# PinataFarms/FEARTracker

Hardware: NVIDIA H100
Metric: FEAR-XS frames/sec (track + decode, batch 256 per GPU) (higher is better)
Workload: dtype f32

## Files before the change

### feartracker_b200/csrc/kernels_tc.cuh

```cuda
#pragma once
#include <cuda_runtime.h>
#include <stdlib.h>

#include <initializer_list>

#include "tc_common.cuh"

namespace fear {
namespace tc {

constexpr int kCorrChunk = 32;
constexpr int kCorrABytes = 128 * 128;
constexpr int kCorrBBytes = 64 * 128;
constexpr int kTcThreads = 288;
constexpr int kTcConsumers = 256;

__device__ __forceinline__ void consumer_sync() { asm volatile("bar.sync 1, 256;" ::: "memory"); }

constexpr int kCorrStages = 3;
constexpr int kCorrStageBytes = kCorrABytes + 2 * kCorrBBytes;
constexpr int kCorrSmemBytes = kCorrStages * kCorrStageBytes + 1024  + 256 ;

__global__ void __launch_bounds__(kTcThreads, 1)
corr_tc_kernel(const __grid_constant__ CUtensorMap tmA, const __grid_constant__ CUtensorMap tmB,
               float* __restrict__ cat, int z_mod) {
  extern __shared__ uint8_t smem_raw[];
  uint8_t* smem = smem_raw + ((1024u - (smem_u32(smem_raw) & 1023u)) & 1023u);
  uint64_t* full = reinterpret_cast<uint64_t*>(smem + kCorrStages * kCorrStageBytes);
  uint64_t* empty = full + kCorrStages;
  const int warp = threadIdx.x >> 5, lane = threadIdx.x & 31;
  constexpr int kChunks = 256 / kCorrChunk;
  if (threadIdx.x == 0) {
    prefetch_tmap(&tmA);
    prefetch_tmap(&tmB);
    for (int s = 0; s < kCorrStages; ++s) {
      mbar_init(&full[s], 1);
      mbar_init(&empty[s], 8);
    }
    fence_mbar_init();
  }
  __syncthreads();
  pdl_trigger();
  pdl_wait();
  const int frame = blockIdx.x >> 1, half = blockIdx.x & 1;
  const int arow = frame * 256 + half * 128;
  auto st_x = [&](int s) { return smem + s * kCorrStageBytes; };
  auto st_z = [&](int s) { return smem + s * kCorrStageBytes + kCorrABytes; };

  if (warp == 8) {
    if (lane == 0) {
      const int brow = z_mod ? (frame % z_mod) * 64 : 0;
      for (int c = 0; c < kChunks; ++c) {
        const int stage = c % kCorrStages;
        mbar_wait_backoff(&empty[stage], (uint32_t)(((c / kCorrStages) & 1) ^ 1));
        mbar_arrive_expect_tx(&full[stage], kCorrABytes + kCorrBBytes);
        tma_load_2d(st_x(stage), &tmA, &full[stage], c * kCorrChunk, arow);
        tma_load_2d(st_z(stage), &tmB, &full[stage], c * kCorrChunk, brow);
      }
    }
    return;
  }
  const int wg = warp >> 2, r0 = wg * 64 + (warp & 3) * 16 + (lane >> 2), t = lane & 3;
  float accm[32], accc[32];
#pragma unroll
  for (int i = 0; i < 32; ++i) accm[i] = accc[i] = 0.f;
  for (int c = 0; c < kChunks; ++c) {
    const int stage = c % kCorrStages;
    mbar_wait(&full[stage], (uint32_t)((c / kCorrStages) & 1));
    float4* zh = reinterpret_cast<float4*>(st_z(stage));
    float4* zl = reinterpret_cast<float4*>(st_z(stage) + kCorrBBytes);
#pragma unroll
    for (int i = 0; i < kCorrBBytes / 16 / kTcConsumers; ++i) {
      const float4 v = zh[threadIdx.x + i * kTcConsumers];
      float4 h, l;
      split_tf32_trunc(v.x, h.x, l.x);
      split_tf32_trunc(v.y, h.y, l.y);
      split_tf32_trunc(v.z, h.z, l.z);
      split_tf32_trunc(v.w, h.w, l.w);
      zh[threadIdx.x + i * kTcConsumers] = h;
      zl[threadIdx.x + i * kTcConsumers] = l;
    }
    fence_proxy_async_smem();
    consumer_sync();
    uint32_t hi[4][4], lo[4][4];
    load_a_frags(st_x(stage), r0, t, hi, lo);
    const uint32_t bh = smem_u32(zh), bl = smem_u32(zl);
    wg_fence();
#pragma unroll
    for (int j = 0; j < 4; ++j) mma3<64>(accm, accc, hi[j], lo[j], bh + j * 32, bl + j * 32);
    wg_commit();
    wg_wait();
    __syncwarp();
    if (lane == 0) mbar_arrive(&empty[stage]);
  }
  float* out = cat + (long long)(arow + r0) * 320 + 256 + 2 * t;
#pragma unroll
  for (int i = 0; i < 8; ++i) {
    *reinterpret_cast<float2*>(out + 8 * i) = make_float2(accm[4 * i] + accc[4 * i], accm[4 * i + 1] + accc[4 * i + 1]);
    *reinterpret_cast<float2*>(out + 8 * 320 + 8 * i) =
        make_float2(accm[4 * i + 2] + accc[4 * i + 2], accm[4 * i + 3] + accc[4 * i + 3]);
  }
}

inline int init_pw();

inline int init() {
  int dev = 0;
  if (cudaGetDevice(&dev) != cudaSuccess) return -1;
  cudaDeviceProp p;
  if (cudaGetDeviceProperties(&p, dev) != cudaSuccess) return -1;
  DeviceState& st = dev_state();
  st.num_sms = p.multiProcessorCount;
  st.inited = true;
  if (resolve_driver()) return 0;
  if (cudaFuncSetAttribute(corr_tc_kernel, cudaFuncAttributeMaxDynamicSharedMemorySize, kCorrSmemBytes) != cudaSuccess) {
    cudaGetLastError();
    return 0;
  }
  if (init_pw()) return 0;
  st.tc_ready = true;
  return 0;
}

inline int launch_corr(cudaStream_t s, const float* zt, int Bz, float* cat, int B, int groups) {
  if (!available()) return -20;
  CUtensorMap tmA, tmB;
  const int frames = B * groups;
  int r;
  r = make_tmap_2d(&tmA, cat, (uint64_t)frames * 256, 320, 320, 128, kCorrChunk);
  if (r) return r;
  r = make_tmap_2d(&tmB, zt, (uint64_t)Bz * 64, 256, 256, 64, kCorrChunk);
  if (r) return r;
  if (launch_pdl(corr_tc_kernel, dim3(frames * 2), dim3(kTcThreads), kCorrSmemBytes, s, tmA, tmB, cat, Bz == 1 ? 0 : B) !=
      cudaSuccess)
    return -23;
  return 0;
}

struct PwParams {
  const float* bias;
  const float* R;
  float* C;
  int ldr, ldc;
  int M, N, num_n_tiles, num_chunks, last_ksteps, relu, stages, stage_bytes;
  int dw_relu, dw_bias;
  int box_bytes;
};

template <int NT, int DWK, int MW = 16>
__global__ void __launch_bounds__(kTcThreads, 1)
pw_tc_kernel(const __grid_constant__ CUtensorMap tmA, const __grid_constant__ CUtensorMap tmWh,
             const __grid_constant__ CUtensorMap tmWl, const __grid_constant__ CUtensorMap tmDW,
             const __grid_constant__ CUtensorMap tmDB, const PwParams p) {
  extern __shared__ uint8_t smem_raw[];
  uint8_t* smem = smem_raw + ((1024u - (smem_u32(smem_raw) & 1023u)) & 1023u);
  const int S = p.stages;
  uint64_t* full = reinterpret_cast<uint64_t*>(smem + S * p.stage_bytes);
  uint64_t* empty = full + S;
  const int warp = threadIdx.x >> 5, lane = threadIdx.x & 31;
  constexpr int w_bytes = NT * 128;
  if (threadIdx.x == 0) {
    prefetch_tmap(&tmA);
    prefetch_tmap(&tmWh);
    prefetch_tmap(&tmWl);
    for (int s = 0; s < S; ++s) {
      mbar_init(&full[s], 1);
      mbar_init(&empty[s], 8);
    }
    fence_mbar_init();
  }
  __syncthreads();
  pdl_trigger();
  pdl_wait();

  const int mt = blockIdx.x / p.num_n_tiles, nt = blockIdx.x - mt * p.num_n_tiles;
  auto a_tile = [&](int s) { return smem + s * p.stage_bytes; };
  auto w_hi = [&](int s) { return smem + s * p.stage_bytes + kCorrABytes; };
  auto w_lo = [&](int s) { return w_hi(s) + w_bytes; };
  auto dw_box = [&](int s) { return w_lo(s) + w_bytes; };
  auto dw_wts = [&](int s) { return dw_box(s) + p.box_bytes; };
  auto dw_bia = [&](int s) { return dw_wts(s) + DWK * DWK * 128; };

  if (warp == 8) {
    if (lane == 0) {
      constexpr int th = 128 / MW, tpf = MW / th;
      for (int c = 0; c < p.num_chunks; ++c) {
        const int stage = c % S;
        mbar_wait_backoff(&empty[stage], (uint32_t)(((c / S) & 1) ^ 1));
        if constexpr (DWK > 0) {
          mbar_arrive_expect_tx(&full[stage], 2 * w_bytes + p.box_bytes + DWK * DWK * 128 + (p.dw_bias ? 128 : 0));
          tma_load_4d(dw_box(stage), &tmA, &full[stage], c * 32, -(DWK / 2), (mt % tpf) * th - DWK / 2, mt / tpf);
          tma_load_2d(dw_wts(stage), &tmDW, &full[stage], c * 32, 0);
          if (p.dw_bias) tma_load_2d(dw_bia(stage), &tmDB, &full[stage], c * 32, 0);
        } else {
          mbar_arrive_expect_tx(&full[stage], kCorrABytes + 2 * w_bytes);
          tma_load_2d(a_tile(stage), &tmA, &full[stage], c * 32, mt * 128);
        }
        tma_load_2d(w_hi(stage), &tmWh, &full[stage], c * 32, nt * NT);
        tma_load_2d(w_lo(stage), &tmWl, &full[stage], c * 32, nt * NT);
      }
    }
    return;
  }

  const int wg = warp >> 2, r0 = wg * 64 + (warp & 3) * 16 + (lane >> 2), t = lane & 3;
  float accm[NT / 2], accc[NT / 2];
#pragma unroll
  for (int i = 0; i < NT / 2; ++i) accm[i] = accc[i] = 0.f;
  for (int c = 0; c < p.num_chunks; ++c) {
    const int stage = c % S;
    mbar_wait(&full[stage], (uint32_t)((c / S) & 1));
    if constexpr (DWK > 0) {
      constexpr int K = DWK, TX = 8, NIN = TX + K - 1, IW = MW + K - 1, PXN = MW / TX;
      typedef unsigned long long U2;
      const int c2 = threadIdx.x & 15, pos = threadIdx.x >> 4;
      const int x0 = (pos % PXN) * TX, y0 = pos / PXN;
      const U2* in2 = reinterpret_cast<const U2*>(dw_box(stage)) + (y0 * IW + x0) * 16 + c2;
      const U2* w2 = reinterpret_cast<const U2*>(dw_wts(stage)) + c2;
      const U2 bias2 = p.dw_bias ? reinterpret_cast<const U2*>(dw_bia(stage))[c2] : 0ull;
      U2 acc[TX];
#pragma unroll
      for (int i = 0; i < TX; ++i) acc[i] = bias2;
#pragma unroll
      for (int ky = 0; ky < K; ++ky) {
        U2 v[NIN];
#pragma unroll
        for (int i = 0; i < NIN; ++i) v[i] = in2[(ky * IW + i) * 16];
#pragma unroll
        for (int kx = 0; kx < K; ++kx) {
          const U2 k = w2[(ky * K + kx) * 16];
#pragma unroll
          for (int i = 0; i < TX; ++i) ffma2(acc[i], v[i + kx], k);
        }
      }
      uint8_t* at = a_tile(stage);
#pragma unroll
      for (int i = 0; i < TX; ++i) {
        float2 v = make_float2(__uint_as_float((uint32_t)acc[i]), __uint_as_float((uint32_t)(acc[i] >> 32)));
        if (p.dw_relu) {
          v.x = fmaxf(v.x, 0.f);
          v.y = fmaxf(v.y, 0.f);
        }
        const int R = y0 * MW + x0 + i;
        *reinterpret_cast<float2*>(at + R * 128 + (((c2 >> 1) ^ (R & 7)) << 4) + ((c2 & 1) << 3)) = v;
      }
      consumer_sync();
    }
    uint32_t hi[4][4], lo[4][4];
    load_a_frags(a_tile(stage), r0, t, hi, lo);
    const uint32_t bh = smem_u32(w_hi(stage)), bl = smem_u32(w_lo(stage));
    const int ksteps = (c == p.num_chunks - 1) ? p.last_ksteps : 4;
    wg_fence();
#pragma unroll
    for (int j = 0; j < 4; ++j)
      if (j < ksteps) mma3<NT>(accm, accc, hi[j], lo[j], bh + j * 32, bl + j * 32);
    wg_commit();
    wg_wait();
    __syncwarp();
    if (lane == 0) mbar_arrive(&empty[stage]);
  }

  const int n0 = nt * NT + 2 * t;
#pragma unroll
  for (int hrow = 0; hrow < 2; ++hrow) {
    const long long grow = (long long)mt * 128 + r0 + hrow * 8;
    if (grow >= p.M) continue;
#pragma unroll
    for (int i = 0; i < NT / 8; ++i) {
      const int col = n0 + 8 * i;
      if (col >= p.N) continue;
      float2 o = make_float2(accm[4 * i + 2 * hrow] + accc[4 * i + 2 * hrow], accm[4 * i + 2 * hrow + 1] + accc[4 * i + 2 * hrow + 1]);
      float2 b = p.bias ? __ldg(reinterpret_cast<const float2*>(p.bias + col)) : make_float2(0.f, 0.f);
      if (p.R) {
        const float2 rr = __ldg(reinterpret_cast<const float2*>(p.R + grow * p.ldr + col));
        b.x += rr.x;
        b.y += rr.y;
      }
      o.x += b.x;
      o.y += b.y;
      if (p.relu) {
        o.x = fmaxf(o.x, 0.f);
        o.y = fmaxf(o.y, 0.f);
      }
      *reinterpret_cast<float2*>(p.C + grow * p.ldc + col) = o;
    }
  }
}

constexpr int kPwMaxSmem = 232448 - 1024;
constexpr int kPwMaxStages = 3;

inline int pw_tile_n(int N) {
  const int Np = (N + 15) & ~15;
  const int tiles = (Np + 127) / 128;
  const int need = (Np + tiles - 1) / tiles;
  for (int nt : {16, 32, 48, 64, 96, 112, 128})
    if (nt >= need) return nt;
  return 0;
}

inline bool pw_supported(int cin, int cout) { return available() && cin % 8 == 0 && cout % 8 == 0; }

#define FEAR_PW_FOR_NT(X) X(16) X(32) X(48) X(64) X(96) X(112) X(128)

constexpr int kPwNarrowNT = 32;
inline int pw_tile_n_one_chunk(int N) {
  const int Np = (N + 15) & ~15;
  const int tiles = (Np + kPwNarrowNT - 1) / kPwNarrowNT;
  const int need = (Np + tiles - 1) / tiles;
  return need <= 16 ? 16 : 32;
}

inline int init_pw() {
  cudaError_t e = cudaSuccess;
#define FEAR_PW_ATTR(NT_)                                                                                                  \
  if (e == cudaSuccess) e = cudaFuncSetAttribute(pw_tc_kernel<NT_, 0>, cudaFuncAttributeMaxDynamicSharedMemorySize, kPwMaxSmem);     \
  if (e == cudaSuccess) e = cudaFuncSetAttribute(pw_tc_kernel<NT_, 3, 16>, cudaFuncAttributeMaxDynamicSharedMemorySize, kPwMaxSmem); \
  if (e == cudaSuccess) e = cudaFuncSetAttribute(pw_tc_kernel<NT_, 5, 16>, cudaFuncAttributeMaxDynamicSharedMemorySize, kPwMaxSmem); \
  if (e == cudaSuccess) e = cudaFuncSetAttribute(pw_tc_kernel<NT_, 3, 32>, cudaFuncAttributeMaxDynamicSharedMemorySize, kPwMaxSmem); \
  if (e == cudaSuccess) e = cudaFuncSetAttribute(pw_tc_kernel<NT_, 5, 32>, cudaFuncAttributeMaxDynamicSharedMemorySize, kPwMaxSmem);
  FEAR_PW_FOR_NT(FEAR_PW_ATTR)
#undef FEAR_PW_ATTR
  if (e != cudaSuccess) {
    cudaGetLastError();
    return -1;
  }
  return 0;
}

inline int launch_pw(cudaStream_t s, const float* A, int lda, const float* w_hi, const float* w_lo, const float* bias,
                     const float* R, int ldr, float* C, int ldc, int M, int N, int K, int relu) {
  if (!available()) return -20;
  PwParams p;
  p.bias = bias;
  p.R = R;
  p.C = C;
  p.ldr = ldr;
  p.ldc = ldc;
  p.M = M;
  p.N = N;
  p.num_chunks = (K + 31) / 32;
  const int NT = p.num_chunks == 1 ? pw_tile_n_one_chunk(N) : pw_tile_n(N);
  if (!NT) return -21;
  p.num_n_tiles = (((N + 15) & ~15) + NT - 1) / NT;
  p.last_ksteps = ((K - 32 * (p.num_chunks - 1)) + 7) / 8;
  p.relu = relu;
  p.dw_relu = p.dw_bias = p.box_bytes = 0;
  p.stage_bytes = kCorrABytes + 2 * NT * 128;
  p.stages = p.num_chunks < kPwMaxStages ? p.num_chunks : kPwMaxStages;
  CUtensorMap tmA, tmWh, tmWl;
  int r = make_tmap_2d(&tmA, A, (uint64_t)M, (uint64_t)K, (uint64_t)lda, 128, 32);
  if (r) return r;
  r = make_tmap_2d(&tmWh, w_hi, (uint64_t)N, (uint64_t)K, (uint64_t)K, NT, 32);
  if (r) return r;
  r = make_tmap_2d(&tmWl, w_lo, (uint64_t)N, (uint64_t)K, (uint64_t)K, NT, 32);
  if (r) return r;
  const int tiles = ((M + 127) / 128) * p.num_n_tiles;
  const size_t smem_bytes = (size_t)p.stages * p.stage_bytes + 1024 + 256;
  cudaError_t e = cudaErrorInvalidValue;
  switch (NT) {
#define FEAR_PW_CASE(NT_)                                                                                                     \
  case NT_:                                                                                                                   \
    e = launch_pdl(pw_tc_kernel<NT_, 0>, dim3(tiles), dim3(kTcThreads), smem_bytes, s, tmA, tmWh, tmWl, tmA, tmA, p); \
    break;
    FEAR_PW_FOR_NT(FEAR_PW_CASE)
#undef FEAR_PW_CASE
  }
  return e == cudaSuccess ? 0 : -23;
}

inline int launch_pw_dw(cudaStream_t s, const float* X, int B, int dw_k, const float* dw_w, const float* dw_b, int dw_relu,
                        const float* w_hi, const float* w_lo, const float* bias, const float* R, int ldr, float* C,
                        int ldc, int N, int K, int relu, int map_w = 16) {
  if (!available()) return -20;
  if ((dw_k != 3 && dw_k != 5) || K % 4 || (map_w != 16 && map_w != 32)) return 1;
  PwParams p;
  const int M = B * map_w * map_w;
  p.bias = bias;
  p.R = R;
  p.C = C;
  p.ldr = ldr;
  p.ldc = ldc;
  p.M = M;
  p.N = N;
  p.num_chunks = (K + 31) / 32;
  const int NT = pw_tile_n(N);
  if (!NT) return 1;
  p.num_n_tiles = (((N + 15) & ~15) + NT - 1) / NT;
  p.last_ksteps = ((K - 32 * (p.num_chunks - 1)) + 7) / 8;
  p.relu = relu;
  p.dw_relu = dw_relu;
  p.dw_bias = dw_b != nullptr;
  const int ih = 128 / map_w + dw_k - 1, iw = map_w + dw_k - 1;
  p.box_bytes = ih * iw * 128;
  p.stage_bytes = (kCorrABytes + 2 * NT * 128 + p.box_bytes + dw_k * dw_k * 128 + 128 + 1023) & ~1023;
  p.stages = p.num_chunks < 2 ? 1 : 2;
  const size_t smem_bytes = (size_t)p.stages * p.stage_bytes + 1024 + 256;
  if ((int)smem_bytes > kPwMaxSmem) return 1;
  CUtensorMap tmX, tmWh, tmWl, tmDW, tmDB;
  int r = make_tmap_nhwc(&tmX, X, (uint64_t)B, (uint64_t)map_w, (uint64_t)map_w, (uint64_t)K, 32, iw, ih);
  if (r) return r;
  r = make_tmap_2d(&tmWh, w_hi, (uint64_t)N, (uint64_t)K, (uint64_t)K, NT, 32);
  if (r) return r;
  r = make_tmap_2d(&tmWl, w_lo, (uint64_t)N, (uint64_t)K, (uint64_t)K, NT, 32);
  if (r) return r;
  r = make_tmap_2d_plain(&tmDW, dw_w, (uint64_t)dw_k * dw_k, (uint64_t)K, dw_k * dw_k, 32);
  if (r) return r;
  if (dw_b) {
    r = make_tmap_2d_plain(&tmDB, dw_b, 1, (uint64_t)K, 1, 32);
    if (r) return r;
  } else {
    tmDB = tmDW;
  }
  const int tiles = (M / 128) * p.num_n_tiles;
  cudaError_t e = cudaErrorInvalidValue;
#define FEAR_PW_DW_LAUNCH(NT_, K_, MW_) \
  e = launch_pdl(pw_tc_kernel<NT_, K_, MW_>, dim3(tiles), dim3(kTcThreads), smem_bytes, s, tmX, tmWh, tmWl, tmDW, tmDB, p)
  switch (NT) {
#define FEAR_PW_CASE(NT_)                                \
  case NT_:                                              \
    if (map_w == 16) {                                   \
      if (dw_k == 5) FEAR_PW_DW_LAUNCH(NT_, 5, 16);      \
      else FEAR_PW_DW_LAUNCH(NT_, 3, 16);                \
    } else {                                             \
      if (dw_k == 5) FEAR_PW_DW_LAUNCH(NT_, 5, 32);      \
      else FEAR_PW_DW_LAUNCH(NT_, 3, 32);                \
    }                                                    \
    break;
    FEAR_PW_FOR_NT(FEAR_PW_CASE)
#undef FEAR_PW_CASE
  }
#undef FEAR_PW_DW_LAUNCH
  return e == cudaSuccess ? 0 : -23;
}

}
}
```

### feartracker_b200/csrc/tc_common.cuh

```cuda
#pragma once
#include <cuda.h>
#include <cuda_runtime.h>
#include <stdint.h>
#include <string.h>

#include <mutex>
#include <set>
#include <string>
#include <unordered_map>

namespace fear {
namespace tc {

typedef CUresult (*PFN_encodeTiled)(CUtensorMap*, CUtensorMapDataType, cuuint32_t, void*, const cuuint64_t*,
                                    const cuuint64_t*, const cuuint32_t*, const cuuint32_t*, CUtensorMapInterleave,
                                    CUtensorMapSwizzle, CUtensorMapL2promotion, CUtensorMapFloatOOBfill);

inline PFN_encodeTiled& encode_fn() {
  static PFN_encodeTiled fn = nullptr;
  return fn;
}

inline int resolve_driver() {
  if (encode_fn()) return 0;
  void* p = nullptr;
  cudaDriverEntryPointQueryResult q;
  cudaError_t e = cudaGetDriverEntryPoint("cuTensorMapEncodeTiled", &p, cudaEnableDefault, &q);
  if (e != cudaSuccess || q != cudaDriverEntryPointSuccess || !p) return -10;
  encode_fn() = (PFN_encodeTiled)p;
  return 0;
}

struct DeviceState {
  bool inited = false;
  bool tc_ready = false;
  int num_sms = 0;
  std::set<const void*> attrs;
};
inline std::mutex& state_mutex() {
  static std::mutex m;
  return m;
}
inline DeviceState& dev_state() {
  static DeviceState st[64];
  int d = 0;
  cudaGetDevice(&d);
  return st[d & 63];
}
inline bool available() { return dev_state().tc_ready; }
inline int num_sms() { return dev_state().num_sms; }
inline bool attr_needed(const void* fn) {
  std::lock_guard<std::mutex> lock(state_mutex());
  return dev_state().attrs.insert(fn).second;
}

struct TmapKey {
  uint64_t v[16];
  bool operator==(const TmapKey& o) const { return memcmp(v, o.v, sizeof(v)) == 0; }
};
struct TmapKeyHash {
  size_t operator()(const TmapKey& k) const {
    uint64_t h = 1469598103934665603ull;
    for (uint64_t x : k.v) {
      h ^= x;
      h *= 1099511628211ull;
    }
    return (size_t)h;
  }
};
inline int encode_cached(CUtensorMap* m, CUtensorMapDataType dt, uint32_t rank, const void* base, const cuuint64_t* dims,
                         const cuuint64_t* strides, const cuuint32_t* box, CUtensorMapSwizzle sw,
                         CUtensorMapL2promotion promo) {
  if (resolve_driver()) return -10;
  static thread_local std::unordered_map<TmapKey, CUtensorMap, TmapKeyHash> cache;
  TmapKey k;
  memset(&k, 0, sizeof(k));
  k.v[0] = (uint64_t)(uintptr_t)base;
  k.v[1] = ((uint64_t)dt << 32) | ((uint64_t)rank << 16) | ((uint64_t)sw << 8) | (uint64_t)promo;
  for (uint32_t i = 0; i < rank; ++i) {
    k.v[2 + i] = dims[i];
    k.v[7 + i] = (i + 1 < rank) ? strides[i] : 0;
    k.v[12 + (i >> 1)] |= (uint64_t)box[i] << (32 * (i & 1));
  }
  auto it = cache.find(k);
  if (it != cache.end()) {
    *m = it->second;
    return 0;
  }
  cuuint32_t estr[5] = {1, 1, 1, 1, 1};
  CUresult r = encode_fn()(m, dt, rank, const_cast<void*>(base), dims, strides, box, estr, CU_TENSOR_MAP_INTERLEAVE_NONE, sw,
                           promo, CU_TENSOR_MAP_FLOAT_OOB_FILL_NONE);
  if (r != CUDA_SUCCESS) return -11;
  if (cache.size() > 8192) cache.clear();
  cache.emplace(k, *m);
  return 0;
}

inline int make_tmap_2d(CUtensorMap* m, const float* base, uint64_t rows, uint64_t cols, uint64_t pitch_floats,
                        uint32_t box_rows, uint32_t box_cols) {
  cuuint64_t dims[2] = {cols, rows};
  cuuint64_t strides[1] = {pitch_floats * sizeof(float)};
  cuuint32_t box[2] = {box_cols, box_rows};
  CUtensorMapSwizzle sw = (box_cols * 4 == 128)  ? CU_TENSOR_MAP_SWIZZLE_128B
                          : (box_cols * 4 == 64) ? CU_TENSOR_MAP_SWIZZLE_64B
                                                 : CU_TENSOR_MAP_SWIZZLE_NONE;
  return encode_cached(m, CU_TENSOR_MAP_DATA_TYPE_FLOAT32, 2, base, dims, strides, box, sw,
                       CU_TENSOR_MAP_L2_PROMOTION_L2_256B);
}

inline int make_tmap_nhwc(CUtensorMap* m, const float* base, uint64_t B, uint64_t H, uint64_t W, uint64_t C,
                          uint32_t box_c, uint32_t box_w, uint32_t box_h,
                          CUtensorMapSwizzle sw = CU_TENSOR_MAP_SWIZZLE_NONE) {
  cuuint64_t dims[4] = {C, W, H, B};
  cuuint64_t strides[3] = {C * sizeof(float), W * C * sizeof(float), H * W * C * sizeof(float)};
  cuuint32_t box[4] = {box_c, box_w, box_h, 1};
  return encode_cached(m, CU_TENSOR_MAP_DATA_TYPE_FLOAT32, 4, base, dims, strides, box, sw,
                       CU_TENSOR_MAP_L2_PROMOTION_L2_128B);
}

inline int make_tmap_3d(CUtensorMap* m, CUtensorMapDataType dt, const void* base, uint64_t d0, uint64_t d1, uint64_t d2,
                        uint64_t stride1_bytes, uint64_t stride2_bytes, uint32_t b0, uint32_t b1, uint32_t b2) {
  cuuint64_t dims[3] = {d0, d1, d2};
  cuuint64_t strides[2] = {stride1_bytes, stride2_bytes};
  cuuint32_t box[3] = {b0, b1, b2};
  return encode_cached(m, dt, 3, base, dims, strides, box, CU_TENSOR_MAP_SWIZZLE_NONE, CU_TENSOR_MAP_L2_PROMOTION_L2_128B);
}

inline int make_tmap_2d_plain(CUtensorMap* m, const float* base, uint64_t rows, uint64_t cols, uint32_t box_rows,
                              uint32_t box_cols) {
  cuuint64_t dims[2] = {cols, rows};
  cuuint64_t strides[1] = {cols * sizeof(float)};
  cuuint32_t box[2] = {box_cols, box_rows};
  return encode_cached(m, CU_TENSOR_MAP_DATA_TYPE_FLOAT32, 2, base, dims, strides, box, CU_TENSOR_MAP_SWIZZLE_NONE,
                       CU_TENSOR_MAP_L2_PROMOTION_L2_128B);
}

inline bool& pdl_enabled() {
  static bool on = true;
  return on;
}
template <typename... KArgs, typename... Args>
inline cudaError_t launch_pdl(void (*kern)(KArgs...), dim3 grid, dim3 block, size_t smem, cudaStream_t s, Args&&... args) {
  cudaLaunchConfig_t cfg = {};
  cfg.gridDim = grid;
  cfg.blockDim = block;
  cfg.dynamicSmemBytes = smem;
  cfg.stream = s;
  cudaLaunchAttribute attr[1];
  attr[0].id = cudaLaunchAttributeProgrammaticStreamSerialization;
  attr[0].val.programmaticStreamSerializationAllowed = 1;
  cudaStreamCaptureStatus cap = cudaStreamCaptureStatusNone;
  const bool use = pdl_enabled() && cudaStreamIsCapturing(s, &cap) == cudaSuccess && cap == cudaStreamCaptureStatusNone;
  cfg.attrs = attr;
  cfg.numAttrs = use ? 1 : 0;
  return cudaLaunchKernelEx(&cfg, kern, static_cast<KArgs>(args)...);
}

__device__ __forceinline__ uint32_t smem_u32(const void* p) { return (uint32_t)__cvta_generic_to_shared(p); }

__device__ __forceinline__ bool elect_one() {
  uint32_t pred = 0;
  asm volatile(
      "{\n\t"
      ".reg .pred P;\n\t"
      "elect.sync _|P, 0xffffffff;\n\t"
      "selp.u32 %0, 1, 0, P;\n\t"
      "}\n"
      : "=r"(pred));
  return pred != 0;
}

__device__ __forceinline__ void mbar_init(uint64_t* bar, uint32_t count) {
  asm volatile("mbarrier.init.shared::cta.b64 [%0], %1;" ::"r"(smem_u32(bar)), "r"(count) : "memory");
}
__device__ __forceinline__ void fence_mbar_init() { asm volatile("fence.mbarrier_init.release.cluster;" ::: "memory"); }
__device__ __forceinline__ void mbar_arrive(uint64_t* bar) {
  asm volatile("mbarrier.arrive.shared::cta.b64 _, [%0];" ::"r"(smem_u32(bar)) : "memory");
}
__device__ __forceinline__ void mbar_arrive_expect_tx(uint64_t* bar, uint32_t bytes) {
  asm volatile("mbarrier.arrive.expect_tx.shared::cta.b64 _, [%0], %1;" ::"r"(smem_u32(bar)), "r"(bytes) : "memory");
}
__device__ __forceinline__ bool mbar_try_wait(uint64_t* bar, uint32_t parity) {
  uint32_t ok;
  asm volatile(
      "{\n\t"
      ".reg .pred P;\n\t"
      "mbarrier.try_wait.parity.shared::cta.b64 P, [%1], %2;\n\t"
      "selp.u32 %0, 1, 0, P;\n\t"
      "}\n"
      : "=r"(ok)
      : "r"(smem_u32(bar)), "r"(parity)
      : "memory");
  return ok != 0;
}
__device__ __forceinline__ void mbar_wait(uint64_t* bar, uint32_t parity) {
#pragma unroll 1
  for (uint32_t spin = 0; spin < (1u << 26); ++spin)
    if (mbar_try_wait(bar, parity)) return;
  __trap();
}

__device__ __forceinline__ void mbar_wait_backoff(uint64_t* bar, uint32_t parity) {
  if (mbar_try_wait(bar, parity)) return;
#pragma unroll 1
  for (uint32_t spin = 0; spin < (1u << 24); ++spin) {
    __nanosleep(64);
    if (mbar_try_wait(bar, parity)) return;
  }
  __trap();
}

__device__ __forceinline__ void fence_proxy_async_smem() { asm volatile("fence.proxy.async.shared::cta;" ::: "memory"); }

__device__ __forceinline__ void prefetch_tmap(const CUtensorMap* m) {
  asm volatile("prefetch.tensormap [%0];" ::"l"(reinterpret_cast<uint64_t>(m)) : "memory");
}
__device__ __forceinline__ void tma_load_2d(void* smem_dst, const CUtensorMap* m, uint64_t* bar, int32_t c0, int32_t c1) {
  asm volatile(
      "cp.async.bulk.tensor.2d.shared::cluster.global.mbarrier::complete_tx::bytes [%0], [%1, {%3, %4}], [%2];"
      ::"r"(smem_u32(smem_dst)), "l"(reinterpret_cast<uint64_t>(m)), "r"(smem_u32(bar)), "r"(c0), "r"(c1)
      : "memory");
}
__device__ __forceinline__ void tma_load_3d(void* smem_dst, const CUtensorMap* m, uint64_t* bar, int32_t c0, int32_t c1,
                                            int32_t c2) {
  asm volatile(
      "cp.async.bulk.tensor.3d.shared::cluster.global.mbarrier::complete_tx::bytes [%0], [%1, {%3, %4, %5}], [%2];"
      ::"r"(smem_u32(smem_dst)), "l"(reinterpret_cast<uint64_t>(m)), "r"(smem_u32(bar)), "r"(c0), "r"(c1), "r"(c2)
      : "memory");
}
__device__ __forceinline__ void tma_load_4d(void* smem_dst, const CUtensorMap* m, uint64_t* bar, int32_t c0, int32_t c1,
                                            int32_t c2, int32_t c3) {
  asm volatile(
      "cp.async.bulk.tensor.4d.shared::cluster.global.mbarrier::complete_tx::bytes [%0], [%1, {%3, %4, %5, %6}], [%2];"
      ::"r"(smem_u32(smem_dst)), "l"(reinterpret_cast<uint64_t>(m)), "r"(smem_u32(bar)), "r"(c0), "r"(c1), "r"(c2),
      "r"(c3)
      : "memory");
}
__device__ __forceinline__ void tma_prefetch_4d(const CUtensorMap* m, int32_t c0, int32_t c1, int32_t c2, int32_t c3) {
  asm volatile("cp.async.bulk.prefetch.tensor.4d.L2.global.tile [%0, {%1, %2, %3, %4}];" ::"l"(reinterpret_cast<uint64_t>(m)),
               "r"(c0), "r"(c1), "r"(c2), "r"(c3)
               : "memory");
}
__device__ __forceinline__ void tma_store_2d(const CUtensorMap* m, const void* smem_src, int32_t c0, int32_t c1) {
  asm volatile("cp.async.bulk.tensor.2d.global.shared::cta.bulk_group [%0, {%2, %3}], [%1];" ::"l"(
                   reinterpret_cast<uint64_t>(m)),
               "r"(smem_u32(smem_src)), "r"(c0), "r"(c1)
               : "memory");
}
__device__ __forceinline__ void tma_store_commit() { asm volatile("cp.async.bulk.commit_group;" ::: "memory"); }
template <int N>
__device__ __forceinline__ void tma_store_wait_read() {
  asm volatile("cp.async.bulk.wait_group.read %0;" ::"n"(N) : "memory");
}
template <int N>
__device__ __forceinline__ void tma_store_wait() {
  asm volatile("cp.async.bulk.wait_group %0;" ::"n"(N) : "memory");
}

struct __align__(16) F4 {
  unsigned long long lo, hi;
};
__device__ __forceinline__ void ffma2(unsigned long long& acc, unsigned long long a, unsigned long long b) {
  const float x = fmaf(__uint_as_float((uint32_t)a), __uint_as_float((uint32_t)b), __uint_as_float((uint32_t)acc));
  const float y = fmaf(__uint_as_float((uint32_t)(a >> 32)), __uint_as_float((uint32_t)(b >> 32)), __uint_as_float((uint32_t)(acc >> 32)));
  acc = (unsigned long long)__float_as_uint(x) | ((unsigned long long)__float_as_uint(y) << 32);
}
__device__ __forceinline__ unsigned long long pack2(uint32_t lo, uint32_t hi) {
  return (unsigned long long)lo | ((unsigned long long)hi << 32);
}
__device__ __forceinline__ float4 f4_to_float4(const F4& v) {
  float4 r;
  r.x = __uint_as_float((unsigned)(v.lo & 0xffffffffull));
  r.y = __uint_as_float((unsigned)(v.lo >> 32));
  r.z = __uint_as_float((unsigned)(v.hi & 0xffffffffull));
  r.w = __uint_as_float((unsigned)(v.hi >> 32));
  return r;
}

__device__ __forceinline__ void pdl_trigger() { asm volatile("griddepcontrol.launch_dependents;" ::: "memory"); }
__device__ __forceinline__ void pdl_wait() { asm volatile("griddepcontrol.wait;" ::: "memory"); }

__device__ __forceinline__ void wg_fence() { asm volatile("wgmma.fence.sync.aligned;" ::: "memory"); }
__device__ __forceinline__ void wg_commit() { asm volatile("wgmma.commit_group.sync.aligned;" ::: "memory"); }
__device__ __forceinline__ void wg_wait() { asm volatile("wgmma.wait_group.sync.aligned 0;" ::: "memory"); }

#define FEAR_WG_D8(d, o) "+f"(d[o]), "+f"(d[o + 1]), "+f"(d[o + 2]), "+f"(d[o + 3]), "+f"(d[o + 4]), "+f"(d[o + 5]), "+f"(d[o + 6]), "+f"(d[o + 7])
template <int N>
__device__ __forceinline__ void wgmma_tf32(float* d, const uint32_t (&a)[4], uint64_t bdesc);
template <>
__device__ __forceinline__ void wgmma_tf32<16>(float* d, const uint32_t (&a)[4], uint64_t bdesc) {
  asm volatile(
      "{\n\t.reg .pred p;\n\tsetp.ne.b32 p, 1, 0;\n\t"
      "wgmma.mma_async.sync.aligned.m64n16k8.f32.tf32.tf32 {%0, %1, %2, %3, %4, %5, %6, %7}, {%8, %9, %10, %11}, %12, p, 1, 1;\n\t}\n"
      : FEAR_WG_D8(d, 0)
      : "r"(a[0]), "r"(a[1]), "r"(a[2]), "r"(a[3]), "l"(bdesc));
}
template <>
__device__ __forceinline__ void wgmma_tf32<32>(float* d, const uint32_t (&a)[4], uint64_t bdesc) {
  asm volatile(
      "{\n\t.reg .pred p;\n\tsetp.ne.b32 p, 1, 0;\n\t"
      "wgmma.mma_async.sync.aligned.m64n32k8.f32.tf32.tf32 {%0, %1, %2, %3, %4, %5, %6, %7, %8, %9, %10, %11, %12, %13, %14, %15}, "
      "{%16, %17, %18, %19}, %20, p, 1, 1;\n\t}\n"
      : FEAR_WG_D8(d, 0), FEAR_WG_D8(d, 8)
      : "r"(a[0]), "r"(a[1]), "r"(a[2]), "r"(a[3]), "l"(bdesc));
}
template <>
__device__ __forceinline__ void wgmma_tf32<64>(float* d, const uint32_t (&a)[4], uint64_t bdesc) {
  asm volatile(
      "{\n\t.reg .pred p;\n\tsetp.ne.b32 p, 1, 0;\n\t"
      "wgmma.mma_async.sync.aligned.m64n64k8.f32.tf32.tf32 {%0, %1, %2, %3, %4, %5, %6, %7, %8, %9, %10, %11, %12, %13, %14, %15, "
      "%16, %17, %18, %19, %20, %21, %22, %23, %24, %25, %26, %27, %28, %29, %30, %31}, {%32, %33, %34, %35}, %36, p, 1, 1;\n\t}\n"
      : FEAR_WG_D8(d, 0), FEAR_WG_D8(d, 8), FEAR_WG_D8(d, 16), FEAR_WG_D8(d, 24)
      : "r"(a[0]), "r"(a[1]), "r"(a[2]), "r"(a[3]), "l"(bdesc));
}
#undef FEAR_WG_D8

__device__ __forceinline__ uint64_t wg_desc_k_sw128(uint32_t smem_addr) {
  uint64_t d = (uint64_t)((smem_addr & 0x3FFFF) >> 4);
  d |= (uint64_t)1 << 16;
  d |= (uint64_t)(1024 >> 4) << 32;
  d |= (uint64_t)1 << 62;
  return d;
}

template <int NT>
__device__ __forceinline__ void mma3(float* main, float* corr, const uint32_t (&ah)[4], const uint32_t (&al)[4],
                                     uint32_t bh, uint32_t bl) {
  static_assert(NT % 16 == 0 && NT <= 128, "tile width");
  constexpr int n0 = NT >= 64 ? 64 : (NT >= 32 ? 32 : 16);
  wgmma_tf32<n0>(main, ah, wg_desc_k_sw128(bh));
  wgmma_tf32<n0>(corr, ah, wg_desc_k_sw128(bl));
  wgmma_tf32<n0>(corr, al, wg_desc_k_sw128(bh));
  if constexpr (NT > n0) mma3<NT - n0>(main + n0 / 2, corr + n0 / 2, ah, al, bh + n0 * 128, bl + n0 * 128);
}

__device__ __forceinline__ void load_a_frags(const uint8_t* tile, int r0, int t, uint32_t (&hi)[4][4], uint32_t (&lo)[4][4]) {
  const int g = r0 & 7;
#pragma unroll
  for (int j = 0; j < 4; ++j)
#pragma unroll
    for (int e = 0; e < 4; ++e) {
      const int row = r0 + (e & 1) * 8, ch = 2 * j + (e >> 1);
      const float v = *reinterpret_cast<const float*>(tile + row * 128 + ((ch ^ g) << 4) + t * 4);
      const uint32_t h = __float_as_uint(v) & 0xFFFFE000u;
      hi[j][e] = h;
      lo[j][e] = __float_as_uint(v - __uint_as_float(h));
    }
}

inline float host_rna_tf32(float v) {
  uint32_t u;
  memcpy(&u, &v, 4);
  u = (u + 0x1000u) & 0xFFFFE000u;
  float r;
  memcpy(&r, &u, 4);
  return r;
}

__device__ __forceinline__ void split_tf32(float v, float& hi, float& lo) {
  uint32_t h, l;
  asm("cvt.rna.tf32.f32 %0, %1;" : "=r"(h) : "f"(v));
  hi = __uint_as_float(h);
  const float r = v - hi;
  asm("cvt.rna.tf32.f32 %0, %1;" : "=r"(l) : "f"(r));
  lo = __uint_as_float(l);
}

__device__ __forceinline__ void split_tf32_trunc(float v, float& hi, float& lo) {
  hi = __uint_as_float(__float_as_uint(v) & 0xFFFFE000u);
  lo = v - hi;
}

}
}
```

Before: 32640.

## Make pointwise TC kernel persistent with warp-specialized producer and async wgmma overlap

Rewrites the pointwise tensor-core GEMM kernel as a persistent kernel, with the grid capped at the SM count and a loop over tiles. It uses a full producer warpgroup with setmaxnreg register rebalancing and keeps one wgmma group in flight, so the next chunk's A-fragment loads overlap the current MMAs. The fused depthwise path now writes into two double-buffered A buffers outside the TMA stages, and the stage count grows up to 4 based on the shared memory available. Single-chunk GEMMs are routed to a separate narrow non-persistent kernel. The intent is to remove per-tile launch and prologue overhead and to hide TMA and MMA latency, at the cost of more complexity and higher smem pressure.

```diff
diff --git a/feartracker_b200/csrc/kernels_tc.cuh b/feartracker_b200/csrc/kernels_tc.cuh
--- a/feartracker_b200/csrc/kernels_tc.cuh
+++ b/feartracker_b200/csrc/kernels_tc.cuh
@@ -142,16 +142,212 @@
   const float* R;
   float* C;
   int ldr, ldc;
-  int M, N, num_n_tiles, num_chunks, last_ksteps, relu, stages, stage_bytes;
+  int M, N, num_n_tiles, num_tiles, num_chunks, last_ksteps, relu, stages, stage_bytes;
   int dw_relu, dw_bias;
   int box_bytes;
 };
 
+constexpr int kPwThreads = 384;
+constexpr int kPwProducerRegs = 40, kPwConsumerRegs = 232;
+
+template <int NT, int KS>
+__device__ __forceinline__ void mma3_chunk(float* accm, float* accc, const uint32_t (&hi)[4][4], const uint32_t (&lo)[4][4],
+                                           uint32_t bh, uint32_t bl) {
+#pragma unroll
+  for (int j = 0; j < KS; ++j) mma3<NT>(accm, accc, hi[j], lo[j], bh + j * 32, bl + j * 32);
+}
+
+template <int K, int MW>
+__device__ __forceinline__ void dw_chunk(const uint8_t* box, const uint8_t* wts, const uint8_t* bia, uint8_t* at, int ct,
+                                         int dw_bias, int dw_relu) {
+  constexpr int TX = 8, NIN = TX + K - 1, IW = MW + K - 1, PXN = MW / TX;
+  typedef unsigned long long U2;
+  const int c2 = ct & 15, pos = ct >> 4;
+  const int x0 = (pos % PXN) * TX, y0 = pos / PXN;
+  const U2* in2 = reinterpret_cast<const U2*>(box) + (y0 * IW + x0) * 16 + c2;
+  const U2* w2 = reinterpret_cast<const U2*>(wts) + c2;
+  const U2 bias2 = dw_bias ? reinterpret_cast<const U2*>(bia)[c2] : 0ull;
+  U2 acc[TX];
+#pragma unroll
+  for (int i = 0; i < TX; ++i) acc[i] = bias2;
+#pragma unroll
+  for (int ky = 0; ky < K; ++ky) {
+    U2 v[NIN];
+#pragma unroll
+    for (int i = 0; i < NIN; ++i) v[i] = in2[(ky * IW + i) * 16];
+#pragma unroll
+    for (int kx = 0; kx < K; ++kx) {
+      const U2 k = w2[(ky * K + kx) * 16];
+#pragma unroll
+      for (int i = 0; i < TX; ++i) ffma2(acc[i], v[i + kx], k);
+    }
+  }
+#pragma unroll
+  for (int i = 0; i < TX; ++i) {
+    float2 v = make_float2(__uint_as_float((uint32_t)acc[i]), __uint_as_float((uint32_t)(acc[i] >> 32)));
+    if (dw_relu) {
+      v.x = fmaxf(v.x, 0.f);
+      v.y = fmaxf(v.y, 0.f);
+    }
+    const int R = y0 * MW + x0 + i;
+    *reinterpret_cast<float2*>(at + R * 128 + (((c2 >> 1) ^ (R & 7)) << 4) + ((c2 & 1) << 3)) = v;
+  }
+}
+
+template <int NT>
+__device__ __forceinline__ void pw_epilogue(const PwParams& p, const float* accm, const float* accc, int mt, int nt, int r0,
+                                            int t) {
+  const int n0 = nt * NT + 2 * t;
+#pragma unroll
+  for (int hrow = 0; hrow < 2; ++hrow) {
+    const long long grow = (long long)mt * 128 + r0 + hrow * 8;
+    if (grow >= p.M) continue;
+#pragma unroll
+    for (int i = 0; i < NT / 8; ++i) {
+      const int col = n0 + 8 * i;
+      if (col >= p.N) continue;
+      float2 o = make_float2(accm[4 * i + 2 * hrow] + accc[4 * i + 2 * hrow], accm[4 * i + 2 * hrow + 1] + accc[4 * i + 2 * hrow + 1]);
+      float2 b = p.bias ? __ldg(reinterpret_cast<const float2*>(p.bias + col)) : make_float2(0.f, 0.f);
+      if (p.R) {
+        const float2 rr = __ldg(reinterpret_cast<const float2*>(p.R + grow * p.ldr + col));
+        b.x += rr.x;
+        b.y += rr.y;
+      }
+      o.x += b.x;
+      o.y += b.y;
+      if (p.relu) {
+        o.x = fmaxf(o.x, 0.f);
+        o.y = fmaxf(o.y, 0.f);
+      }
+      *reinterpret_cast<float2*>(p.C + grow * p.ldc + col) = o;
+    }
+  }
+}
+
 template <int NT, int DWK, int MW = 16>
-__global__ void __launch_bounds__(kTcThreads, 1)
+__global__ void __launch_bounds__(kPwThreads, 1)
 pw_tc_kernel(const __grid_constant__ CUtensorMap tmA, const __grid_constant__ CUtensorMap tmWh,
              const __grid_constant__ CUtensorMap tmWl, const __grid_constant__ CUtensorMap tmDW,
              const __grid_constant__ CUtensorMap tmDB, const PwParams p) {
+  extern __shared__ uint8_t smem_raw[];
+  uint8_t* smem = smem_raw + ((1024u - (smem_u32(smem_raw) & 1023u)) & 1023u);
+  const int S = p.stages;
+  constexpr int a_bufs = DWK > 0 ? 2 : 0;
+  uint64_t* full = reinterpret_cast<uint64_t*>(smem + S * p.stage_bytes + a_bufs * kCorrABytes);
+  uint64_t* empty = full + S;
+  constexpr int w_bytes = NT * 128;
+  if (threadIdx.x == 0) {
+    prefetch_tmap(&tmA);
+    prefetch_tmap(&tmWh);
+    prefetch_tmap(&tmWl);
+    for (int s = 0; s < S; ++s) {
+      mbar_init(&full[s], 1);
+      mbar_init(&empty[s], 8);
+    }
+    fence_mbar_init();
+  }
+  __syncthreads();
+  pdl_trigger();
+  pdl_wait();
+
+  auto a_tile = [&](int s) { return smem + s * p.stage_bytes; };
+  auto a_buf = [&](int b) { return smem + S * p.stage_bytes + b * kCorrABytes; };
+  auto w_hi = [&](int s) { return smem + s * p.stage_bytes + (DWK > 0 ? 0 : kCorrABytes); };
+  auto w_lo = [&](int s) { return w_hi(s) + w_bytes; };
+  auto dw_box = [&](int s) { return w_lo(s) + w_bytes; };
+  auto dw_wts = [&](int s) { return dw_box(s) + p.box_bytes; };
+  auto dw_bia = [&](int s) { return dw_wts(s) + DWK * DWK * 128; };
+
+  const int wg = __shfl_sync(0xffffffffu, (int)threadIdx.x / 128, 0);
+  if (wg == 0) {
+    setmaxnreg_dec<kPwProducerRegs>();
+    if (threadIdx.x == 0) {
+      constexpr int th = 128 / MW, tpf = MW / th;
+      int stage = 0;
+      uint32_t phase = 0;
+      for (int tile = blockIdx.x; tile < p.num_tiles; tile += gridDim.x) {
+        const int mt = tile / p.num_n_tiles, nt = tile - mt * p.num_n_tiles;
+        for (int c = 0; c < p.num_chunks; ++c) {
+          mbar_wait_backoff(&empty[stage], phase ^ 1);
+          if constexpr (DWK > 0) {
+            mbar_arrive_expect_tx(&full[stage], 2 * w_bytes + p.box_bytes + DWK * DWK * 128 + (p.dw_bias ? 128 : 0));
+            tma_load_4d(dw_box(stage), &tmA, &full[stage], c * 32, -(DWK / 2), (mt % tpf) * th - DWK / 2, mt / tpf);
+            tma_load_2d(dw_wts(stage), &tmDW, &full[stage], c * 32, 0);
+            if (p.dw_bias) tma_load_2d(dw_bia(stage), &tmDB, &full[stage], c * 32, 0);
+          } else {
+            mbar_arrive_expect_tx(&full[stage], kCorrABytes + 2 * w_bytes);
+            tma_load_2d(a_tile(stage), &tmA, &full[stage], c * 32, mt * 128);
+          }
+          tma_load_2d(w_hi(stage), &tmWh, &full[stage], c * 32, nt * NT);
+          tma_load_2d(w_lo(stage), &tmWl, &full[stage], c * 32, nt * NT);
+          if (++stage == S) {
+            stage = 0;
+            phase ^= 1;
+          }
+        }
+      }
+    }
+    return;
+  }
+  setmaxnreg_inc<kPwConsumerRegs>();
+
+  const int ct = threadIdx.x - 128, warp = ct >> 5, lane = ct & 31;
+  const int r0 = (warp >> 2) * 64 + (warp & 3) * 16 + (lane >> 2), t = lane & 3;
+  int stage = 0, ab = 0;
+  uint32_t phase = 0;
+  for (int tile = blockIdx.x; tile < p.num_tiles; tile += gridDim.x) {
+    const int mt = tile / p.num_n_tiles, nt = tile - mt * p.num_n_tiles;
+    float accm[NT / 2], accc[NT / 2];
+#pragma unroll
+    for (int i = 0; i < NT / 2; ++i) accm[i] = accc[i] = 0.f;
+    if constexpr (DWK > 0) {
+      mbar_wait(&full[stage], phase);
+      dw_chunk<DWK, MW>(dw_box(stage), dw_wts(stage), dw_bia(stage), a_buf(ab), ct, p.dw_bias, p.dw_relu);
+      consumer_sync();
+    }
+    int prev = 0;
+    for (int c = 0; c < p.num_chunks; ++c) {
+      if constexpr (DWK == 0) mbar_wait(&full[stage], phase);
+      uint32_t hi[4][4], lo[4][4];
+      load_a_frags(DWK > 0 ? a_buf(ab) : a_tile(stage), r0, t, hi, lo);
+      const uint32_t bh = smem_u32(w_hi(stage)), bl = smem_u32(w_lo(stage));
+      const int ksteps = (c == p.num_chunks - 1) ? p.last_ksteps : 4;
+      wg_fence();
+      if (ksteps == 4) mma3_chunk<NT, 4>(accm, accc, hi, lo, bh, bl);
+      else if (ksteps == 3) mma3_chunk<NT, 3>(accm, accc, hi, lo, bh, bl);
+      else if (ksteps == 2) mma3_chunk<NT, 2>(accm, accc, hi, lo, bh, bl);
+      else mma3_chunk<NT, 1>(accm, accc, hi, lo, bh, bl);
+      wg_commit();
+      if (c > 0) {
+        wg_wait_n<1>();
+        __syncwarp();
+        if (lane == 0) mbar_arrive(&empty[prev]);
+      }
+      prev = stage;
+      if (++stage == S) {
+        stage = 0;
+        phase ^= 1;
+      }
+      if constexpr (DWK > 0) {
+        ab ^= 1;
+        if (c + 1 < p.num_chunks) {
+          mbar_wait(&full[stage], phase);
+          dw_chunk<DWK, MW>(dw_box(stage), dw_wts(stage), dw_bia(stage), a_buf(ab), ct, p.dw_bias, p.dw_relu);
+          consumer_sync();
+        }
+      }
+    }
+    wg_wait_n<0>();
+    __syncwarp();
+    if (lane == 0) mbar_arrive(&empty[prev]);
+    pw_epilogue<NT>(p, accm, accc, mt, nt, r0, t);
+  }
+}
+
+template <int NT>
+__global__ void __launch_bounds__(kTcThreads, 1)
+pw_tc_narrow_kernel(const __grid_constant__ CUtensorMap tmA, const __grid_constant__ CUtensorMap tmWh,
+                    const __grid_constant__ CUtensorMap tmWl, const PwParams p) {
   extern __shared__ uint8_t smem_raw[];
   uint8_t* smem = smem_raw + ((1024u - (smem_u32(smem_raw) & 1023u)) & 1023u);
   const int S = p.stages;
@@ -177,25 +373,14 @@
   auto a_tile = [&](int s) { return smem + s * p.stage_bytes; };
   auto w_hi = [&](int s) { return smem + s * p.stage_bytes + kCorrABytes; };
   auto w_lo = [&](int s) { return w_hi(s) + w_bytes; };
-  auto dw_box = [&](int s) { return w_lo(s) + w_bytes; };
-  auto dw_wts = [&](int s) { return dw_box(s) + p.box_bytes; };
-  auto dw_bia = [&](int s) { return dw_wts(s) + DWK * DWK * 128; };
 
   if (warp == 8) {
     if (lane == 0) {
-      constexpr int th = 128 / MW, tpf = MW / th;
       for (int c = 0; c < p.num_chunks; ++c) {
         const int stage = c % S;
         mbar_wait_backoff(&empty[stage], (uint32_t)(((c / S) & 1) ^ 1));
-        if constexpr (DWK > 0) {
-          mbar_arrive_expect_tx(&full[stage], 2 * w_bytes + p.box_bytes + DWK * DWK * 128 + (p.dw_bias ? 128 : 0));
-          tma_load_4d(dw_box(stage), &tmA, &full[stage], c * 32, -(DWK / 2), (mt % tpf) * th - DWK / 2, mt / tpf);
-          tma_load_2d(dw_wts(stage), &tmDW, &full[stage], c * 32, 0);
-          if (p.dw_bias) tma_load_2d(dw_bia(stage), &tmDB, &full[stage], c * 32, 0);
-        } else {
-          mbar_arrive_expect_tx(&full[stage], kCorrABytes + 2 * w_bytes);
-          tma_load_2d(a_tile(stage), &tmA, &full[stage], c * 32, mt * 128);
-        }
+        mbar_arrive_expect_tx(&full[stage], kCorrABytes + 2 * w_bytes);
+        tma_load_2d(a_tile(stage), &tmA, &full[stage], c * 32, mt * 128);
         tma_load_2d(w_hi(stage), &tmWh, &full[stage], c * 32, nt * NT);
         tma_load_2d(w_lo(stage), &tmWl, &full[stage], c * 32, nt * NT);
       }
@@ -210,42 +395,6 @@
   for (int c = 0; c < p.num_chunks; ++c) {
     const int stage = c % S;
     mbar_wait(&full[stage], (uint32_t)((c / S) & 1));
-    if constexpr (DWK > 0) {
-      constexpr int K = DWK, TX = 8, NIN = TX + K - 1, IW = MW + K - 1, PXN = MW / TX;
-      typedef unsigned long long U2;
-      const int c2 = threadIdx.x & 15, pos = threadIdx.x >> 4;
-      const int x0 = (pos % PXN) * TX, y0 = pos / PXN;
-      const U2* in2 = reinterpret_cast<const U2*>(dw_box(stage)) + (y0 * IW + x0) * 16 + c2;
-      const U2* w2 = reinterpret_cast<const U2*>(dw_wts(stage)) + c2;
-      const U2 bias2 = p.dw_bias ? reinterpret_cast<const U2*>(dw_bia(stage))[c2] : 0ull;
-      U2 acc[TX];
-#pragma unroll
-      for (int i = 0; i < TX; ++i) acc[i] = bias2;
-#pragma unroll
-      for (int ky = 0; ky < K; ++ky) {
-        U2 v[NIN];
-#pragma unroll
-        for (int i = 0; i < NIN; ++i) v[i] = in2[(ky * IW + i) * 16];
-#pragma unroll
-        for (int kx = 0; kx < K; ++kx) {
-          const U2 k = w2[(ky * K + kx) * 16];
-#pragma unroll
-          for (int i = 0; i < TX; ++i) ffma2(acc[i], v[i + kx], k);
-        }
-      }
-      uint8_t* at = a_tile(stage);
-#pragma unroll
-      for (int i = 0; i < TX; ++i) {
-        float2 v = make_float2(__uint_as_float((uint32_t)acc[i]), __uint_as_float((uint32_t)(acc[i] >> 32)));
-        if (p.dw_relu) {
-          v.x = fmaxf(v.x, 0.f);
-          v.y = fmaxf(v.y, 0.f);
-        }
-        const int R = y0 * MW + x0 + i;
-        *reinterpret_cast<float2*>(at + R * 128 + (((c2 >> 1) ^ (R & 7)) << 4) + ((c2 & 1) << 3)) = v;
-      }
-      consumer_sync();
-    }
     uint32_t hi[4][4], lo[4][4];
     load_a_frags(a_tile(stage), r0, t, hi, lo);
     const uint32_t bh = smem_u32(w_hi(stage)), bl = smem_u32(w_lo(stage));
@@ -259,36 +408,17 @@
     __syncwarp();
     if (lane == 0) mbar_arrive(&empty[stage]);
   }
-
-  const int n0 = nt * NT + 2 * t;
-#pragma unroll
-  for (int hrow = 0; hrow < 2; ++hrow) {
-    const long long grow = (long long)mt * 128 + r0 + hrow * 8;
-    if (grow >= p.M) continue;
-#pragma unroll
-    for (int i = 0; i < NT / 8; ++i) {
-      const int col = n0 + 8 * i;
-      if (col >= p.N) continue;
-      float2 o = make_float2(accm[4 * i + 2 * hrow] + accc[4 * i + 2 * hrow], accm[4 * i + 2 * hrow + 1] + accc[4 * i + 2 * hrow + 1]);
-      float2 b = p.bias ? __ldg(reinterpret_cast<const float2*>(p.bias + col)) : make_float2(0.f, 0.f);
-      if (p.R) {
-        const float2 rr = __ldg(reinterpret_cast<const float2*>(p.R + grow * p.ldr + col));
-        b.x += rr.x;
-        b.y += rr.y;
-      }
-      o.x += b.x;
-      o.y += b.y;
-      if (p.relu) {
-        o.x = fmaxf(o.x, 0.f);
-        o.y = fmaxf(o.y, 0.f);
-      }
-      *reinterpret_cast<float2*>(p.C + grow * p.ldc + col) = o;
-    }
-  }
+  pw_epilogue<NT>(p, accm, accc, mt, nt, r0, t);
 }
 
 constexpr int kPwMaxSmem = 232448 - 1024;
-constexpr int kPwMaxStages = 3;
+constexpr int kPwMaxStages = 4;
+constexpr int kPwSmemExtra = 1024  + 256 ;
+
+inline int pw_stages(int stage_bytes, int fixed_bytes) {
+  const int fit = (kPwMaxSmem - kPwSmemExtra - fixed_bytes) / stage_bytes;
+  return fit < kPwMaxStages ? fit : kPwMaxStages;
+}
 
 inline int pw_tile_n(int N) {
   const int Np = (N + 15) & ~15;
@@ -321,12 +451,16 @@
   if (e == cudaSuccess) e = cudaFuncSetAttribute(pw_tc_kernel<NT_, 5, 32>, cudaFuncAttributeMaxDynamicSharedMemorySize, kPwMaxSmem);
   FEAR_PW_FOR_NT(FEAR_PW_ATTR)
 #undef FEAR_PW_ATTR
+  if (e == cudaSuccess) e = cudaFuncSetAttribute(pw_tc_narrow_kernel<16>, cudaFuncAttributeMaxDynamicSharedMemorySize, kPwMaxSmem);
+  if (e == cudaSuccess) e = cudaFuncSetAttribute(pw_tc_narrow_kernel<32>, cudaFuncAttributeMaxDynamicSharedMemorySize, kPwMaxSmem);
   if (e != cudaSuccess) {
     cudaGetLastError();
     return -1;
   }
   return 0;
 }
+
+inline dim3 pw_grid(int tiles) { return dim3(tiles < num_sms() ? tiles : num_sms()); }
 
 inline int launch_pw(cudaStream_t s, const float* A, int lda, const float* w_hi, const float* w_lo, const float* bias,
                      const float* R, int ldr, float* C, int ldc, int M, int N, int K, int relu) {
@@ -340,14 +474,16 @@
   p.M = M;
   p.N = N;
   p.num_chunks = (K + 31) / 32;
-  const int NT = p.num_chunks == 1 ? pw_tile_n_one_chunk(N) : pw_tile_n(N);
+  const bool narrow = p.num_chunks == 1;
+  const int NT = narrow ? pw_tile_n_one_chunk(N) : pw_tile_n(N);
   if (!NT) return -21;
   p.num_n_tiles = (((N + 15) & ~15) + NT - 1) / NT;
+  p.num_tiles = ((M + 127) / 128) * p.num_n_tiles;
   p.last_ksteps = ((K - 32 * (p.num_chunks - 1)) + 7) / 8;
   p.relu = relu;
   p.dw_relu = p.dw_bias = p.box_bytes = 0;
   p.stage_bytes = kCorrABytes + 2 * NT * 128;
-  p.stages = p.num_chunks < kPwMaxStages ? p.num_chunks : kPwMaxStages;
+  p.stages = narrow ? 1 : pw_stages(p.stage_bytes, 0);
   CUtensorMap tmA, tmWh, tmWl;
   int r = make_tmap_2d(&tmA, A, (uint64_t)M, (uint64_t)K, (uint64_t)lda, 128, 32);
   if (r) return r;
@@ -355,13 +491,17 @@
   if (r) return r;
   r = make_tmap_2d(&tmWl, w_lo, (uint64_t)N, (uint64_t)K, (uint64_t)K, NT, 32);
   if (r) return r;
-  const int tiles = ((M + 127) / 128) * p.num_n_tiles;
-  const size_t smem_bytes = (size_t)p.stages * p.stage_bytes + 1024 + 256;
+  const size_t smem_bytes = (size_t)p.stages * p.stage_bytes + kPwSmemExtra;
   cudaError_t e = cudaErrorInvalidValue;
+  if (narrow) {
+    if (NT == 16) e = launch_pdl(pw_tc_narrow_kernel<16>, dim3(p.num_tiles), dim3(kTcThreads), smem_bytes, s, tmA, tmWh, tmWl, p);
+    else e = launch_pdl(pw_tc_narrow_kernel<32>, dim3(p.num_tiles), dim3(kTcThreads), smem_bytes, s, tmA, tmWh, tmWl, p);
+    return e == cudaSuccess ? 0 : -23;
+  }
   switch (NT) {
-#define FEAR_PW_CASE(NT_)                                                                                                     \
-  case NT_:                                                                                                                   \
-    e = launch_pdl(pw_tc_kernel<NT_, 0>, dim3(tiles), dim3(kTcThreads), smem_bytes, s, tmA, tmWh, tmWl, tmA, tmA, p); \
+#define FEAR_PW_CASE(NT_)                                                                                               \
+  case NT_:                                                                                                             \
+    e = launch_pdl(pw_tc_kernel<NT_, 0>, pw_grid(p.num_tiles), dim3(kPwThreads), smem_bytes, s, tmA, tmWh, tmWl, tmA, tmA, p); \
     break;
     FEAR_PW_FOR_NT(FEAR_PW_CASE)
 #undef FEAR_PW_CASE
@@ -387,16 +527,17 @@
   const int NT = pw_tile_n(N);
   if (!NT) return 1;
   p.num_n_tiles = (((N + 15) & ~15) + NT - 1) / NT;
+  p.num_tiles = (M / 128) * p.num_n_tiles;
   p.last_ksteps = ((K - 32 * (p.num_chunks - 1)) + 7) / 8;
   p.relu = relu;
   p.dw_relu = dw_relu;
   p.dw_bias = dw_b != nullptr;
   const int ih = 128 / map_w + dw_k - 1, iw = map_w + dw_k - 1;
   p.box_bytes = ih * iw * 128;
-  p.stage_bytes = (kCorrABytes + 2 * NT * 128 + p.box_bytes + dw_k * dw_k * 128 + 128 + 1023) & ~1023;
-  p.stages = p.num_chunks < 2 ? 1 : 2;
-  const size_t smem_bytes = (size_t)p.stages * p.stage_bytes + 1024 + 256;
-  if ((int)smem_bytes > kPwMaxSmem) return 1;
+  p.stage_bytes = (2 * NT * 128 + p.box_bytes + dw_k * dw_k * 128 + 128 + 1023) & ~1023;
+  if ((p.num_chunks < 2 ? 1 : 2) * (kCorrABytes + p.stage_bytes) + kPwSmemExtra > kPwMaxSmem) return 1;
+  p.stages = pw_stages(p.stage_bytes, 2 * kCorrABytes);
+  const size_t smem_bytes = (size_t)p.stages * p.stage_bytes + 2 * kCorrABytes + kPwSmemExtra;
   CUtensorMap tmX, tmWh, tmWl, tmDW, tmDB;
   int r = make_tmap_nhwc(&tmX, X, (uint64_t)B, (uint64_t)map_w, (uint64_t)map_w, (uint64_t)K, 32, iw, ih);
   if (r) return r;
@@ -412,10 +553,9 @@
   } else {
     tmDB = tmDW;
   }
-  const int tiles = (M / 128) * p.num_n_tiles;
   cudaError_t e = cudaErrorInvalidValue;
 #define FEAR_PW_DW_LAUNCH(NT_, K_, MW_) \
-  e = launch_pdl(pw_tc_kernel<NT_, K_, MW_>, dim3(tiles), dim3(kTcThreads), smem_bytes, s, tmX, tmWh, tmWl, tmDW, tmDB, p)
+  e = launch_pdl(pw_tc_kernel<NT_, K_, MW_>, pw_grid(p.num_tiles), dim3(kPwThreads), smem_bytes, s, tmX, tmWh, tmWl, tmDW, tmDB, p)
   switch (NT) {
 #define FEAR_PW_CASE(NT_)                                \
   case NT_:                                              \
diff --git a/feartracker_b200/csrc/tc_common.cuh b/feartracker_b200/csrc/tc_common.cuh
--- a/feartracker_b200/csrc/tc_common.cuh
+++ b/feartracker_b200/csrc/tc_common.cuh
@@ -283,6 +283,19 @@
 __device__ __forceinline__ void wg_fence() { asm volatile("wgmma.fence.sync.aligned;" ::: "memory"); }
 __device__ __forceinline__ void wg_commit() { asm volatile("wgmma.commit_group.sync.aligned;" ::: "memory"); }
 __device__ __forceinline__ void wg_wait() { asm volatile("wgmma.wait_group.sync.aligned 0;" ::: "memory"); }
+template <int N>
+__device__ __forceinline__ void wg_wait_n() {
+  asm volatile("wgmma.wait_group.sync.aligned %0;" ::"n"(N) : "memory");
+}
+
+template <int REGS>
+__device__ __forceinline__ void setmaxnreg_dec() {
+  asm volatile("setmaxnreg.dec.sync.aligned.u32 %0;" ::"n"(REGS));
+}
+template <int REGS>
+__device__ __forceinline__ void setmaxnreg_inc() {
+  asm volatile("setmaxnreg.inc.sync.aligned.u32 %0;" ::"n"(REGS));
+}
 
 #define FEAR_WG_D8(d, o) "+f"(d[o]), "+f"(d[o + 1]), "+f"(d[o + 2]), "+f"(d[o + 3]), "+f"(d[o + 4]), "+f"(d[o + 5]), "+f"(d[o + 6]), "+f"(d[o + 7])
 template <int N>
```

Result: faster. 36400, median of 6 (+11.5%).
